# bepu/bepuphysics2

Hardware: NVIDIA B200
Metric: constraint-iterations/sec (solver+integrator) (higher is better)
Workload: dtype f32

## Files before the change

bepuphysics2_b200/csrc/bepu_contacts.cuh:

```cuda
#pragma once
#include "bepu_device_math.cuh"

namespace BEPU_NS {

constexpr int kLanes = 32;

struct GlobalRows { const float* ptr; };
struct GlobalAcc { float* ptr; };
struct StagedRows { uint32_t addr, bar, parity; };
struct StagedAcc { uint32_t addr; float* ptr; };
BEPU_DI float lds_f32(uint32_t addr) {
    float v;
    asm("ld.shared.f32 %0, [%1];" : "=f"(v) : "r"(addr));
    return v;
}
BEPU_DI void rows_ready(GlobalRows) {}
BEPU_DI void rows_ready(StagedRows p) {
    asm volatile(
        "{\n"
        ".reg .pred p;\n"
        "MBAR_WAIT:\n"
        "mbarrier.try_wait.parity.shared::cta.b64 p, [%0], %1;\n"
        "@p bra MBAR_DONE;\n"
        "bra MBAR_WAIT;\n"
// ... 12 lines not shown
BEPU_DI void stacc(StagedAcc a, int r, float v) { __stcs(a.ptr + r * kLanes, v); }

BEPU_DI void penetration_apply(const Inertia& iA, const Inertia& iB, V3 normal, V3 angularA, V3 angularB, float impulse, Velocity& vA, Velocity& vB) {
    V3 dLinA = normal * (impulse * iA.inv_mass);
    V3 dAngA = transform(angularA * impulse, iA.t);
    V3 dLinB = normal * (impulse * iB.inv_mass);
    V3 dAngB = transform(angularB * impulse, iB.t);
    vA.lin = vA.lin + dLinA;
    vA.ang = vA.ang + dAngA;
    vB.lin = vB.lin - dLinB;
    vB.ang = vB.ang + dAngB;
}
BEPU_DI void penetration_warm_start(const Inertia& iA, const Inertia& iB, V3 normal, V3 offsetA, V3 offsetB, float accumulated, Velocity& vA, Velocity& vB) {
    penetration_apply(iA, iB, normal, cross(offsetA, normal), cross(normal, offsetB), accumulated, vA, vB);
}
BEPU_DI void penetration_solve(const Inertia& iA, const Inertia& iB, V3 normal, V3 offsetA, V3 offsetB, float depth, const Springiness& sp, float maxRecovery,
                               float inverseDt, float& accumulated, Velocity& vA, Velocity& vB) {
    V3 angularA = cross(offsetA, normal);
    V3 angularB = cross(normal, offsetB);
    float angularA0 = vector_sandwich(angularA, iA.t);
    float angularB0 = vector_sandwich(angularB, iB.t);
    float linear = iA.inv_mass + iB.inv_mass;
    float effectiveMass = sp.effective_mass_cfm_scale / (linear + angularA0 + angularB0);
    float biasVelocity = fmin_ps(depth * inverseDt, fmin_ps(depth * sp.position_error_to_velocity, maxRecovery));
    float csvaLinear = dot(vA.lin, normal);
    float csvaAngular = dot(vA.ang, angularA);
    float negatedCSVBLinear = dot(vB.lin, normal);
    float csvbAngular = dot(vB.ang, angularB);
    float negatedCSI = accumulated * sp.softness_impulse_scale + (csvaLinear - negatedCSVBLinear + csvaAngular + csvbAngular - biasVelocity) * effectiveMass;
    float previous = accumulated;
    accumulated = fmax_ps(0.0f, accumulated - negatedCSI);
    penetration_apply(iA, iB, normal, angularA, angularB, accumulated - previous, vA, vB);
}
BEPU_DI float updated_depth(float dt, V3 contactOffsetA, V3 offsetB, V3 normal, const Velocity& vA, const Velocity& vB, float depth) {
    V3 contactVelocityA = cross(vA.ang, contactOffsetA) + vA.lin;
    V3 contactOffsetB = contactOffsetA - offsetB;
    V3 contactVelocityB = cross(vB.ang, contactOffsetB) + vB.lin;
    float estimatedDepthChangeVelocity = dot(normal, contactVelocityA - contactVelocityB);
    return depth - estimatedDepthChangeVelocity * dt;
}

BEPU_DI void penetration1_apply(const Inertia& iA, V3 normal, V3 angularA, float impulse, Velocity& vA) {
    V3 dLinA = normal * (impulse * iA.inv_mass);
    V3 dAngA = transform(angularA * impulse, iA.t);
    vA.lin = vA.lin + dLinA;
    vA.ang = vA.ang + dAngA;
}
BEPU_DI void penetration1_solve(const Inertia& iA, V3 normal, V3 offsetA, float depth, const Springiness& sp, float maxRecovery, float inverseDt, float& accumulated,
                                Velocity& vA) {
    V3 angularA = cross(offsetA, normal);
    float angularA0 = vector_sandwich(angularA, iA.t);
    float effectiveMass = sp.effective_mass_cfm_scale / (iA.inv_mass + angularA0);
    float biasVelocity = fmin_ps(depth * inverseDt, fmin_ps(depth * sp.position_error_to_velocity, maxRecovery));
    float csvaLinear = dot(vA.lin, normal);
    float csvaAngular = dot(vA.ang, angularA);
    float negatedCSI = accumulated * sp.softness_impulse_scale + (csvaLinear + csvaAngular - biasVelocity) * effectiveMass;
    float previous = accumulated;
    accumulated = fmax_ps(0.0f, accumulated - negatedCSI);
    penetration1_apply(iA, normal, angularA, accumulated - previous, vA);
}
BEPU_DI float updated_depth1(float dt, V3 contactOffset, V3 normal, const Velocity& v, float depth) {
    V3 contactVelocity = cross(v.ang, contactOffset) + v.lin;
    return depth - dot(normal, contactVelocity) * dt;
}

struct TangentJacobians { M23 linearA, angularA, angularB; };
BEPU_DI TangentJacobians tangent_jacobians(V3 tX, V3 tY, V3 offsetA, V3 offsetB) {
    TangentJacobians j;
    j.linearA = {tX, tY};
    j.angularA = {cross(offsetA, tX), cross(offsetA, tY)};
    j.angularB = {cross(tX, offsetB), cross(tY, offsetB)};
    return j;
}
BEPU_DI void tangent_apply(const TangentJacobians& j, const Inertia& iA, const Inertia& iB, V2 impulse, Velocity& vA, Velocity& vB) {
// ... 120 lines not shown
            V3 offset = ldrow3(p, 4 * i);
            penetration_warm_start(iA, iB, normal, offset, offset - offsetB, ldacc(a, 2 + i), vA, vB);
        }
        twist_apply(normal, iA, iB, ldacc(a, N + 2), vA, vB);
    }
    template <class PR, class AR> BEPU_DI static void solve(const Inertia& iA, const Inertia& iB, float dt, float inverseDt, PR p, AR a, Velocity& vA, Velocity& vB) {
        V3 normal = ldrow3(p, L::kNormal), offsetB = ldrow3(p, L::kOffsetB);
        float friction = ldrow(p, L::kFriction), maxRecovery = ldrow(p, L::kMaxRecovery);
        Springiness sp = compute_springiness(ldrow(p, L::kAngularFrequency), ldrow(p, L::kTwiceDampingRatio), dt);
        if constexpr (N > 1) {
            V3 offs[N];
            float depths[N];
#pragma unroll
            for (int i = 0; i < N; ++i) { offs[i] = ldrow3(p, 4 * i); depths[i] = ldrow(p, 4 * i + 3); }
            const V3 centerA = friction_center<N>(offs, depths);
            float penSum = 0.0f, twistSum = 0.0f;
#pragma unroll 1
            for (int i = 0; i < N; ++i) {
                V3 offset = ldrow3(p, 4 * i);
                float pen = ldacc(a, 2 + i);
                penetration_solve(iA, iB, normal, offset, offset - offsetB, ldrow(p, 4 * i + 3), sp, maxRecovery, inverseDt, pen, vA, vB);
                stacc(a, 2 + i, pen);
                const float lever = pen * distance(centerA, offset);
                penSum = i == 0 ? pen : penSum + pen;
                twistSum = i == 0 ? lever : twistSum + lever;
            }
            V3 x, z;
            build_orthonormal_basis(normal, x, z);
            V2 tangent{ldacc(a, 0), ldacc(a, 1)};
            float twist = ldacc(a, N + 2);
            const float premultiplied = (1.0f / N) * friction;
            tangent_solve(x, z, centerA, centerA - offsetB, iA, iB, premultiplied * penSum, tangent, vA, vB);
            twist_solve(normal, iA, iB, premultiplied * twistSum, twist, vA, vB);
            stacc(a, 0, tangent.x);
            stacc(a, 1, tangent.y);
            stacc(a, N + 2, twist);
        } else
        {
        V3 offs[N];
        float depths[N], pen[N];
#pragma unroll
        for (int i = 0; i < N; ++i) { offs[i] = ldrow3(p, 4 * i); depths[i] = ldrow(p, 4 * i + 3); pen[i] = ldacc(a, 2 + i); }
#pragma unroll
// ... 54 lines not shown
        tangent1_apply(M23{x, z}, M23{cross(centerA, x), cross(centerA, z)}, iA, V2{ldacc(a, 0), ldacc(a, 1)}, vA);
#pragma unroll 1
        for (int i = 0; i < N; ++i) penetration1_apply(iA, normal, cross(ldrow3(p, 4 * i), normal), ldacc(a, 2 + i), vA);
        twist1_apply(normal, iA, ldacc(a, N + 2), vA);
    }
    template <class PR, class AR> BEPU_DI static void solve(const Inertia& iA, float dt, float inverseDt, PR p, AR a, Velocity& vA) {
        V3 normal = ldrow3(p, L::kNormal);
        float friction = ldrow(p, L::kFriction), maxRecovery = ldrow(p, L::kMaxRecovery);
        Springiness sp = compute_springiness(ldrow(p, L::kAngularFrequency), ldrow(p, L::kTwiceDampingRatio), dt);
        if constexpr (N > 1) {
            V3 offs[N];
            float depths[N];
#pragma unroll
            for (int i = 0; i < N; ++i) { offs[i] = ldrow3(p, 4 * i); depths[i] = ldrow(p, 4 * i + 3); }
            const V3 centerA = friction_center<N>(offs, depths);
            float penSum = 0.0f, twistSum = 0.0f;
#pragma unroll 1
            for (int i = 0; i < N; ++i) {
                V3 offset = ldrow3(p, 4 * i);
                float pen = ldacc(a, 2 + i);
                penetration1_solve(iA, normal, offset, ldrow(p, 4 * i + 3), sp, maxRecovery, inverseDt, pen, vA);
                stacc(a, 2 + i, pen);
                const float lever = pen * distance(centerA, offset);
                penSum = i == 0 ? pen : penSum + pen;
                twistSum = i == 0 ? lever : twistSum + lever;
            }
            V3 x, z;
            build_orthonormal_basis(normal, x, z);
            V2 tangent{ldacc(a, 0), ldacc(a, 1)};
            float twist = ldacc(a, N + 2);
            const float premultiplied = (1.0f / N) * friction;
            tangent1_solve(x, z, centerA, iA, premultiplied * penSum, tangent, vA);
            twist1_solve(normal, iA, premultiplied * twistSum, twist, vA);
            stacc(a, 0, tangent.x);
            stacc(a, 1, tangent.y);
            stacc(a, N + 2, twist);
        } else
        {
        V3 offs[N];
        float depths[N], pen[N];
#pragma unroll
        for (int i = 0; i < N; ++i) { offs[i] = ldrow3(p, 4 * i); depths[i] = ldrow(p, 4 * i + 3); pen[i] = ldacc(a, 2 + i); }
#pragma unroll
// ... 139 lines not shown
```

bepuphysics2_b200/csrc/bepu_layout_kernels.h:

```cpp
#pragma once
#include "bepu_device_types.h"

namespace bepucuda {

void launch_split_bodies(const void* raw, int body_count, const BodyBuffers& B, cudaStream_t s);
void launch_merge_bodies(void* raw, int body_count, const BodyBuffers& B, cudaStream_t s);
struct TransposeDesc {
    int32_t* src_refs;
    float* src_prestep;
    float* src_impulses;
    const int32_t* map;
    int32_t src_count;
    int32_t bodies, prestep_rows, impulse_rows;
    int32_t src_bundle_base;
    int32_t flags;
    const int32_t* features_old;
    const int32_t* features_new;
};
constexpr int32_t kDescResidentImpulses = 1, kDescRedistribute = 2;
enum { kTransposeRefs = 1, kTransposePrestep = 2, kTransposeImpulses = 4 };
void launch_transpose_in_all(const DeviceTypeBatch* tbs, const TransposeDesc* descs, const WorkItem* work, int work_count, int W, int what, cudaStream_t s);
void launch_transpose_out_all(const DeviceTypeBatch* tbs, const TransposeDesc* descs, const WorkItem* work, int work_count, int W, int what, cudaStream_t s);
void launch_fill_i32(int32_t* p, size_t n, int32_t v, cudaStream_t s);
void launch_redistribute_impulses(const DeviceTypeBatch* tbs, const TransposeDesc* descs, const WorkItem* work, int work_count, cudaStream_t s);
// ... 12 lines not shown
                           int32_t* error_flag, const TransposeDesc* descs, int W, int32_t* source_bundle_flags, cudaStream_t s);
void launch_collect_stage(const DeviceTypeBatch* tbs, const WorkItem* work, int work_count, const int32_t* bodies_per_type, int stage, const BodyBuffers& B, int32_t* staging,
                          cudaStream_t s);
void launch_apply_stage(const int32_t* staging, int planes, const BodyBuffers& B, cudaStream_t s);
void launch_widen_u8(const uint8_t* in, int32_t* out, size_t n, cudaStream_t s);
void launch_narrow_i32(const int32_t* in, uint8_t* out, size_t n, cudaStream_t s);

void launch_shard_exchange(const uint32_t* pushes, int push_count, int what, const BodyBuffers& B, const ShardPeers& peers, const FrameParams* fp, uint32_t exchange_index,
                           int32_t* error_flag, cudaStream_t s);

void launch_fill_peer_masks(const int32_t* refs, uint32_t* peer_masks, size_t count, const uint8_t* body_masks, int rank, cudaStream_t s);
void launch_boundary_flags(const WorkRecord* records, int count, const int32_t* bodies_per_type, long long peer_delta, uint8_t* flags, cudaStream_t s);

void launch_pack_ref_rows(const WorkRecord* records, int count, int32_t* rows, cudaStream_t s);

constexpr int kLaunchPdl = 1, kLaunchPrefetchRows = 2;
struct SolverLaunchers {
    void (*constraint_stage)(int stage, const WorkRecord* records, const int32_t* ref_rows, int work_count, const BodyBuffers& B, const FrameParams* fp, int launch_flags, cudaStream_t s);
    void (*kinematic_stage)(int stage, const int32_t* kinematics, int count, const BodyBuffers& B, const FrameParams* fp, cudaStream_t s);
    void (*final_pose)(const BodyBuffers& B, const FrameParams* fp, cudaStream_t s);
    void (*constraint_stage_sharded)(int stage, const WorkRecord* records, const int32_t* ref_rows, int work_count, const BodyBuffers& B, const FrameParams* fp, int launch_flags, const ShardPeers& peers,
                                     long long peer_delta, const ShardStage& shard, cudaStream_t s);
};
const SolverLaunchers* get_launchers_bepu_fast();
const SolverLaunchers* get_launchers_bepu_strict();

}
```

bepuphysics2_b200/csrc/bepu_solver_kernels.cu:

```cuda
#include <atomic>
#include "bepu_solver_kernels.cuh"
#include "bepu_layout_kernels.h"

namespace BEPU_NS {

void launch_stage_warm_start_first(const WorkRecord* records, const int32_t* ref_rows, int work_count, const BodyBuffers& B, const FrameParams* fp, int launch_flags, cudaStream_t s);
void launch_stage_warm_start(const WorkRecord* records, const int32_t* ref_rows, int work_count, const BodyBuffers& B, const FrameParams* fp, int launch_flags, cudaStream_t s);
void launch_stage_solve(const WorkRecord* records, const int32_t* ref_rows, int work_count, const BodyBuffers& B, const FrameParams* fp, int launch_flags, cudaStream_t s);
void launch_stage_warm_start_first_sharded(const WorkRecord* records, const int32_t* ref_rows, int work_count, const BodyBuffers& B, const FrameParams* fp, int launch_flags, const ShardPeers& peers, long long peer_delta, const ShardStage& shard, cudaStream_t s);
void launch_stage_warm_start_sharded(const WorkRecord* records, const int32_t* ref_rows, int work_count, const BodyBuffers& B, const FrameParams* fp, int launch_flags, const ShardPeers& peers, long long peer_delta, const ShardStage& shard, cudaStream_t s);
void launch_stage_solve_sharded(const WorkRecord* records, const int32_t* ref_rows, int work_count, const BodyBuffers& B, const FrameParams* fp, int launch_flags, const ShardPeers& peers, long long peer_delta, const ShardStage& shard, cudaStream_t s);

#ifndef BEPU_DEEP_MINB
#define BEPU_DEEP_MINB 12
#endif
constexpr int kDeepBatchBundles = 2400;
template <int STAGE, int MINB>
static void launch_stage_variant(const WorkRecord* records, const int32_t* ref_rows, int work_count, const BodyBuffers& B, const FrameParams* fp, int launch_flags, cudaStream_t s) {
    static std::atomic<bool> carveout_set[64] = {};
    int device = 0;
    cudaGetDevice(&device);
    if (!carveout_set[device & 63]) {
        cudaFuncSetAttribute(constraint_stage_kernel<STAGE, MINB>, cudaFuncAttributePreferredSharedMemoryCarveout, cudaSharedmemCarveoutMaxShared);
        carveout_set[device & 63] = true;
    }
    const unsigned blocks = (unsigned)(((size_t)work_count * 32 + kStageBlockThreads - 1) / kStageBlockThreads);
    cudaLaunchConfig_t cfg{};
    cfg.gridDim = dim3(blocks);
    cfg.blockDim = dim3(kStageBlockThreads);
    cfg.dynamicSmemBytes = 0;
    cfg.stream = s;
    cudaLaunchAttribute attr[1];
    attr[0].id = cudaLaunchAttributeProgrammaticStreamSerialization;
    attr[0].val.programmaticStreamSerializationAllowed = 1;
    cfg.attrs = attr;
    cfg.numAttrs = (launch_flags & bepucuda::kLaunchPdl) ? 1 : 0;
    cudaLaunchKernelEx(&cfg, constraint_stage_kernel<STAGE, MINB>, records, ref_rows, work_count, B, fp, (launch_flags & bepucuda::kLaunchPrefetchRows) ? kStagePrefetchRows : 0);
}
template <int STAGE, int MINB>
static void launch_stage_variant_sharded(const WorkRecord* records, const int32_t* ref_rows, int work_count, const BodyBuffers& B, const FrameParams* fp, int launch_flags, const ShardPeers& peers, long long peer_delta,
                                         const ShardStage& shard, cudaStream_t s) {
    static std::atomic<bool> carveout_set[64] = {};
    int device = 0;
    cudaGetDevice(&device);
    if (!carveout_set[device & 63]) {
        cudaFuncSetAttribute(constraint_stage_kernel_sharded<STAGE, MINB>, cudaFuncAttributePreferredSharedMemoryCarveout, cudaSharedmemCarveoutMaxShared);
        carveout_set[device & 63] = true;
    }
    const unsigned blocks = (unsigned)(((size_t)work_count * 32 + kStageBlockThreads - 1) / kStageBlockThreads);
    cudaLaunchConfig_t cfg{};
    cfg.gridDim = dim3(blocks);
    cfg.blockDim = dim3(kStageBlockThreads);
// ... 88 lines not shown
```

bepuphysics2_b200/csrc/bepu_solver_kernels.cuh:

```cuda
#pragma once
#include "bepu_contacts.cuh"
#include "bepu_joints_more.cuh"
#include "bepu_integration.cuh"
#include "bepu_device_types.h"

namespace BEPU_NS {

using namespace bepucuda;

struct F8 { float a, b, c, d, e, f, g, h; };
#define BEPU_BODY_LD "ld.global.L1::no_allocate.L2::evict_last.v8.f32"
#define BEPU_BODY_ST "st.global.L1::no_allocate.L2::evict_last.v8.f32"
BEPU_DI F8 ld256(const float4* p) {
    F8 r;
    asm volatile(BEPU_BODY_LD " {%0,%1,%2,%3,%4,%5,%6,%7}, [%8];"
                 : "=f"(r.a), "=f"(r.b), "=f"(r.c), "=f"(r.d), "=f"(r.e), "=f"(r.f), "=f"(r.g), "=f"(r.h)
                 : "l"(p)
                 : "memory");
    return r;
}
BEPU_DI void st256(float4* p, float a, float b, float c, float d, float e, float f, float g, float h) {
    asm volatile(BEPU_BODY_ST " [%0], {%1,%2,%3,%4,%5,%6,%7,%8};" ::"l"(p), "f"(a), "f"(b), "f"(c), "f"(d), "f"(e), "f"(f), "f"(g), "f"(h) : "memory");
}
BEPU_DI void load_velocity(const float4* vel, uint32_t i, Velocity& v) {
// ... 3 lines not shown
}
BEPU_DI void store_velocity(float4* vel, uint32_t i, const Velocity& v) { st256(vel + 2 * (size_t)i, v.lin.x, v.lin.y, v.lin.z, 0.0f, v.ang.x, v.ang.y, v.ang.z, 0.0f); }
BEPU_DI void load_inertia(const float4* in, uint32_t i, Inertia& r) {
    const F8 x = ld256(in + 2 * (size_t)i);
    r.t = {x.a, x.b, x.c, x.d, x.e, x.f};
    r.inv_mass = x.g;
}
BEPU_DI void store_inertia(float4* in, uint32_t i, const Inertia& r) { st256(in + 2 * (size_t)i, r.t.xx, r.t.yx, r.t.yy, r.t.zx, r.t.zy, r.t.zz, r.inv_mass, 0.0f); }
BEPU_DI void load_pose(const float4* pose, uint32_t i, V3& pos, Q4& q) {
    const F8 x = ld256(pose + 2 * (size_t)i);
    q = {x.a, x.b, x.c, x.d};
    pos = {x.e, x.f, x.g};
}
BEPU_DI void store_pose(float4* pose, uint32_t i, V3 pos, Q4 q) { st256(pose + 2 * (size_t)i, q.x, q.y, q.z, q.w, pos.x, pos.y, pos.z, 0.0f); }

template <int STAGE, bool NeedsPose>
BEPU_DI void warm_start_body(uint32_t enc, const BodyBuffers& B, const FrameParams& fp, BodyState& b, Velocity& v) {
    const uint32_t idx = enc & kRefIndexMask;
    if (enc & kRefIntegrateBit) {
        Inertia local;
        load_inertia(B.inertia_local, idx, local);
        load_pose(B.pose, idx, b.pos, b.q);
        b.inertia.inv_mass = local.inv_mass;
        if (STAGE == kStageWarmStart) {
            b.pos = b.pos + v.lin * fp.dt;
            Q4 previousOrientation = b.q;
            b.q = integrate_orientation(b.q, v.ang, fp.dt * 0.5f);
            b.inertia.t = rotate_inverse_inertia(local.t, b.q);
            if (fp.angular_mode == 1) integrate_angular_conserve_momentum(previousOrientation, local.t, b.inertia.t, v.ang);
            else if (fp.angular_mode == 2) integrate_angular_gyroscopic(b.q, local.t, v.ang, fp.dt);
            store_pose(B.pose, idx, b.pos, b.q);
        } else {
            b.inertia.t = rotate_inverse_inertia(local.t, b.q);
            if (fp.angular_mode == 1) {
                Q4 previousOrientation = integrate_orientation(b.q, v.ang, fp.dt * -0.5f);
                integrate_angular_conserve_momentum(previousOrientation, local.t, b.inertia.t, v.ang);
            } else if (fp.angular_mode == 2) {
// ... 5 lines not shown
    } else {
        load_inertia(B.inertia_world, idx, b.inertia);
        if (NeedsPose) load_pose(B.pose, idx, b.pos, b.q);
        if (STAGE == kStageWarmStartFirst && fp.angular_mode != 0 && (enc & kRefBundleIntegratesBit) && !(enc & kRefKinematicBit)) {
            Inertia local;
            load_inertia(B.inertia_local, idx, local);
            V3 pos;
            Q4 q;
            load_pose(B.pose, idx, pos, q);
            if (fp.angular_mode == 1) integrate_angular_conserve_momentum(integrate_orientation(q, v.ang, fp.dt * -0.5f), local.t, b.inertia.t, v.ang);
            else integrate_angular_gyroscopic(q, local.t, v.ang, fp.dt);
        }
    }
}
template <int STAGE, bool NeedsPose>
BEPU_DI void gather_for_warm_start(uint32_t enc, const BodyBuffers& B, const FrameParams& fp, BodyState& b, Velocity& v) {
    load_velocity(B.velocity, enc & kRefIndexMask, v);
    warm_start_body<STAGE, NeedsPose>(enc, B, fp, b, v);
}

template <class T, class PR, class AR> BEPU_DI void call_warm_start(const BodyState* b, PR p, AR a, Velocity* v) {
    if constexpr (T::kNeedsPose) T::warm_start(b, p, a, v);
    else if constexpr (T::kBodies == 2) T::warm_start(b[0].inertia, b[1].inertia, p, a, v[0], v[1]);
    else T::warm_start(b[0].inertia, p, a, v[0]);
}
template <class T, class PR, class AR> BEPU_DI void call_solve(const BodyState* b, float dt, float inverseDt, PR p, AR a, Velocity* v) {
    if constexpr (T::kNeedsPose) T::solve(b, dt, inverseDt, p, a, v);
    else if constexpr (T::kBodies == 2) T::solve(b[0].inertia, b[1].inertia, dt, inverseDt, p, a, v[0], v[1]);
    else T::solve(b[0].inertia, dt, inverseDt, p, a, v[0]);
}
template <class T> BEPU_DI void call_incremental(float dt, const Velocity* v, float* p) {
    if constexpr (T::kIncremental) {
        if constexpr (T::kBodies == 2) T::incremental_update(dt, v[0], v[1], p);
// ... 4 lines not shown
BEPU_DI uint32_t ldg_nc_u32(const void* p) {
    uint32_t v;
    asm volatile("ld.global.nc.u32 %0, [%1];" : "=r"(v) : "l"(p));
    return v;
}
BEPU_DI void push_record(float4* const* arrays, uint32_t mask, uint32_t idx, float a, float b, float c, float d, float e, float f, float g, float h) {
    while (mask) {
        const int q = __ffs((int)mask) - 1;
        mask &= mask - 1u;
        float4* dst = arrays[q] + 2 * (size_t)idx;
        dst[0] = make_float4(a, b, c, d);
        dst[1] = make_float4(e, f, g, h);
    }
}
template <class T, int STAGE, bool kSharded, class PR, class AR>
BEPU_DI void run_lane(const int32_t* refs, PR p, AR a, float* p_rw, uint32_t enc0, uint32_t enc1, const BodyBuffers& B, const FrameParams& fp, const ShardPeers* peers = nullptr,
                      long long peer_delta = 0) {
    constexpr int NB = T::kBodies;
    uint32_t enc[NB];
    enc[0] = enc0;
    if constexpr (NB > 1) enc[1] = enc1;
#pragma unroll
    for (int s = 2; s < NB; ++s) enc[s] = (uint32_t)__ldg(refs + s * kLanes);
    uint32_t push_to[kSharded ? NB : 1];
    if constexpr (kSharded) {
#pragma unroll
        for (int s = 0; s < NB; ++s) push_to[s] = peer_delta != 0 ? ldg_nc_u32(refs + peer_delta + s * kLanes) : 0u;
    }
    if ((int32_t)enc[0] == kRefEmpty) return;
    BodyState b[NB];
    Velocity v[NB];
    if constexpr (STAGE == kStageIncremental) {
#pragma unroll
        for (int s = 0; s < NB; ++s) load_velocity(B.velocity, enc[s] & kRefIndexMask, v[s]);
        call_incremental<T>(fp.dt, v, p_rw);
    } else if constexpr (STAGE == kStageSolve) {
#pragma unroll
        for (int s = 0; s < NB; ++s) {
            const uint32_t idx = enc[s] & kRefIndexMask;
            load_velocity(B.velocity, idx, v[s]);
            load_inertia(B.inertia_world, idx, b[s].inertia);
            if (T::kNeedsPose) load_pose(B.pose, idx, b[s].pos, b[s].q);
        }
        rows_ready(p);
        call_solve<T>(b, fp.dt, fp.inverse_dt, p, a, v);
#pragma unroll
        for (int s = 0; s < NB; ++s)
            if (!(enc[s] & kRefKinematicBit)) {
                store_velocity(B.velocity, enc[s] & kRefIndexMask, v[s]);
                if constexpr (kSharded) {
                    const uint32_t mask = push_to[s];
                    if (mask) push_record(peers->velocity, mask, enc[s] & kRefIndexMask, v[s].lin.x, v[s].lin.y, v[s].lin.z, 0.0f, v[s].ang.x, v[s].ang.y, v[s].ang.z, 0.0f);
                }
            }
    } else {
#pragma unroll
        for (int s = 0; s < NB; ++s) gather_for_warm_start<STAGE, T::kNeedsPose>(enc[s], B, fp, b[s], v[s]);
        rows_ready(p);
        call_warm_start<T>(b, p, a, v);
#pragma unroll
        for (int s = 0; s < NB; ++s)
            if (!(enc[s] & kRefKinematicBit)) {
                const uint32_t idx = enc[s] & kRefIndexMask;
                store_velocity(B.velocity, idx, v[s]);
                if constexpr (kSharded) {
                    const uint32_t mask = push_to[s];
                    if (mask) {
                        push_record(peers->velocity, mask, idx, v[s].lin.x, v[s].lin.y, v[s].lin.z, 0.0f, v[s].ang.x, v[s].ang.y, v[s].ang.z, 0.0f);
                        if (enc[s] & kRefIntegrateBit) {
                            const Inertia& in = b[s].inertia;
                            push_record(peers->inertia_world, mask, idx, in.t.xx, in.t.yx, in.t.yy, in.t.zx, in.t.zy, in.t.zz, in.inv_mass, 0.0f);
                            if (STAGE == kStageWarmStart) push_record(peers->pose, mask, idx, b[s].q.x, b[s].q.y, b[s].q.z, b[s].q.w, b[s].pos.x, b[s].pos.y, b[s].pos.z, 0.0f);
                        }
                    }
                }
            }
    }
}
template <class T, int STAGE, class PR, class AR>
BEPU_DI void run_lane(const int32_t* refs, PR p, AR a, float* p_rw, uint32_t enc0, uint32_t enc1, const BodyBuffers& B, const FrameParams& fp) {
    run_lane<T, STAGE, false>(refs, p, a, p_rw, enc0, enc1, B, fp);
}

BEPU_DI int4 ldg_nc_v4(const void* p) {
    int4 v;
    asm volatile("ld.global.nc.v4.s32 {%0,%1,%2,%3}, [%4];" : "=r"(v.x), "=r"(v.y), "=r"(v.z), "=r"(v.w) : "l"(p));
    return v;
}
BEPU_DI WorkRecord load_record(const WorkRecord* r) {
    const int4 lo = ldg_nc_v4(r), hi = ldg_nc_v4(reinterpret_cast<const int4*>(r) + 1);
    WorkRecord w;
    w.refs = reinterpret_cast<int32_t*>((unsigned long long)(unsigned int)lo.x | ((unsigned long long)(unsigned int)lo.y << 32));
    w.prestep = reinterpret_cast<float*>((unsigned long long)(unsigned int)lo.z | ((unsigned long long)(unsigned int)lo.w << 32));
    w.impulses = reinterpret_cast<float*>((unsigned long long)(unsigned int)hi.x | ((unsigned long long)(unsigned int)hi.y << 32));
    w.type_id = hi.z;
    w.live_lanes = hi.w;
    return w;
}

#define BEPU_CONTACT_TYPES(X)                                                                                                     \
    X(0, ConvexOneBody<1>) X(1, ConvexOneBody<2>) X(2, ConvexOneBody<3>) X(3, ConvexOneBody<4>)                                   \
    X(4, ConvexTwoBody<1>) X(5, ConvexTwoBody<2>) X(6, ConvexTwoBody<3>) X(7, ConvexTwoBody<4>)                                   \
    X(8, NonconvexOneBody<2>) X(9, NonconvexOneBody<3>) X(10, NonconvexOneBody<4>)                                                \
    X(15, NonconvexTwoBody<2>) X(16, NonconvexTwoBody<3>) X(17, NonconvexTwoBody<4>)

template <int STAGE, bool kSharded, class PR, class AR>
BEPU_DI void run_bundle_rows(const WorkRecord& rec, int lane, PR p, AR a, uint32_t enc0, uint32_t enc1, const BodyBuffers& B, const FrameParams& fp, const ShardPeers* peers = nullptr,
                             long long peer_delta = 0) {
    const int32_t* refs = rec.refs + lane;
    float* p_rw = rec.prestep + lane;
    switch (rec.type_id) {
#define BEPU_CASE(ID, T) \
    case ID: run_lane<T, STAGE, kSharded>(refs, p, a, p_rw, enc0, enc1, B, fp, peers, peer_delta); break;
        BEPU_CONTACT_TYPES(BEPU_CASE)
        BEPU_JOINT_TYPES(BEPU_CASE)
        BEPU_JOINT_TYPES_MORE(BEPU_CASE)
#undef BEPU_CASE
        default: break;
    }
}
template <int STAGE, class PR, class AR>
BEPU_DI void run_bundle_rows(const WorkRecord& rec, int lane, PR p, AR a, uint32_t enc0, uint32_t enc1, const BodyBuffers& B, const FrameParams& fp) {
    run_bundle_rows<STAGE, false>(rec, lane, p, a, enc0, enc1, B, fp);
}
template <int STAGE>
BEPU_DI void run_bundle(const WorkRecord& rec, int lane, uint32_t enc0, uint32_t enc1, const BodyBuffers& B, const FrameParams& fp) {
    run_bundle_rows<STAGE>(rec, lane, GlobalRows{rec.prestep + lane}, GlobalAcc{rec.impulses + lane}, enc0, enc1, B, fp);
}
template <int STAGE> BEPU_DI void run_bundle(const WorkRecord& rec, int lane, const BodyBuffers& B, const FrameParams& fp) {
    const uint32_t enc0 = ldg_nc_u32(rec.refs + lane), enc1 = ldg_nc_u32(rec.refs + kLanes + lane);
    run_bundle<STAGE>(rec, lane, enc0, enc1, B, fp);
}

struct StageRowCounts { uint8_t prestep[64], impulses[64]; };
__host__ __device__ constexpr StageRowCounts make_stage_row_counts() {
    StageRowCounts c{};
#define BEPU_ROWS(ID, T) c.prestep[ID] = (uint8_t)T::kPrestepRows; c.impulses[ID] = (uint8_t)T::kImpulseRows;
    BEPU_CONTACT_TYPES(BEPU_ROWS)
    BEPU_JOINT_TYPES(BEPU_ROWS)
    BEPU_JOINT_TYPES_MORE(BEPU_ROWS)
#undef BEPU_ROWS
    return c;
}
__constant__ StageRowCounts kStageRowCounts = make_stage_row_counts();
constexpr int kStageSlabRows = 48;
constexpr int kStageSlabBytes = kStageSlabRows * kLanes * 4;

BEPU_DI uint32_t smem_u32(const void* p) { return (uint32_t)__cvta_generic_to_shared(p); }
BEPU_DI void mbar_init(uint32_t bar, uint32_t count) {
    asm volatile("mbarrier.init.shared::cta.b64 [%0], %1;" ::"r"(bar), "r"(count) : "memory");
    asm volatile("fence.mbarrier_init.release.cluster;" ::: "memory");
    asm volatile("fence.proxy.async.shared::cta;" ::: "memory");
// ... 3 lines not shown
    uint64_t policy;
    asm volatile("createpolicy.fractional.L2::evict_first.b64 %0, 1.0;" : "=l"(policy));
    return policy;
}
BEPU_DI void bulk_copy_g2s(uint32_t dst, const void* src, uint32_t bytes, uint32_t bar, uint64_t policy) {
    asm volatile("cp.async.bulk.shared::cluster.global.mbarrier::complete_tx::bytes.L2::cache_hint [%0], [%1], %2, [%3], %4;" ::"r"(dst), "l"(src), "r"(bytes), "r"(bar),
                 "l"(policy)
                 : "memory");
}

#ifndef BEPU_STAGE_BLOCK_THREADS
#define BEPU_STAGE_BLOCK_THREADS 64
#endif
constexpr int kStageBlockThreads = BEPU_STAGE_BLOCK_THREADS;

constexpr int kStagePrefetchRows = 1;
BEPU_DI void shard_announce(const ShardPeers& peers, int lane) {
    if (lane < peers.rank_count && lane != peers.rank)
        asm volatile("red.release.sys.global.add.u64 [%0], 1;" ::"l"(peers.flags[lane] + kShardCounterSlot + peers.rank) : "memory");
}
BEPU_DI void shard_wait(const ShardPeers& peers, int lane, uint32_t solve_index, uint32_t exchange_point, int32_t* error_flag) {
    if (lane < peers.rank_count && lane != peers.rank) {
        const unsigned long long* mine = peers.flags[peers.rank];
        const unsigned long long* targets = mine + kShardTargetSlot + (size_t)lane * kShardMaxExchanges;
        const unsigned long long want = (unsigned long long)solve_index * targets[kShardMaxExchanges - 1] + targets[exchange_point];
        unsigned long long seen;
        unsigned int spins = 0;
        do {
            asm volatile("ld.acquire.sys.global.u64 %0, [%1];" : "=l"(seen) : "l"(mine + kShardCounterSlot + lane) : "memory");
        } while (seen < want && ++spins < 100000000u);
        if (seen < want) atomicExch(error_flag, 5);
    }
    __syncwarp();
}
template <int STAGE, bool kSharded>
BEPU_DI void constraint_stage_body(const WorkRecord* __restrict__ records, const int32_t* __restrict__ ref_rows, int work_count, const BodyBuffers& B, const FrameParams* __restrict__ fpp, int flags, const ShardPeers* peers,
                                   long long peer_delta, const ShardStage* shard = nullptr) {
    constexpr bool kStaged = STAGE != kStageIncremental;
    constexpr int kWarps = kStageBlockThreads / 32;
    __shared__ __align__(128) float slab[kStaged ? kWarps * kStageSlabRows * kLanes : 1];
    __shared__ __align__(8) unsigned long long bars[kWarps];
    const int warp_in_block = threadIdx.x >> 5;
    const int global_warp = (blockIdx.x * kStageBlockThreads + threadIdx.x) >> 5;
    const int lane = threadIdx.x & 31;
    WorkRecord rec{};
    uint32_t enc0 = (uint32_t)kRefEmpty, enc1 = 0;
    const int warp = global_warp;
    const bool active = warp < work_count;
    const uint32_t slab_addr = kStaged ? smem_u32(slab) + warp_in_block * kStageSlabBytes : 0;
    const uint32_t bar = smem_u32(&bars[warp_in_block]);
    const bool early_rows = kStaged && (flags & kStagePrefetchRows);
    uint32_t prestep_bytes = 0, impulse_bytes = 0;
    if (active) {
        rec = load_record(records + warp);
        if constexpr (kStaged) {
            prestep_bytes = kStageRowCounts.prestep[rec.type_id] * (kLanes * 4);
            impulse_bytes = kStageRowCounts.impulses[rec.type_id] * (kLanes * 4);
            if (lane == 0) {
                mbar_init(bar, 1);
                if (early_rows) {
                    const uint64_t policy = l2_evict_first_policy();
                    mbar_expect_tx(bar, prestep_bytes + impulse_bytes);
                    bulk_copy_g2s(slab_addr, rec.prestep, prestep_bytes, bar, policy);
                    bulk_copy_g2s(slab_addr + prestep_bytes, rec.impulses, impulse_bytes, bar, policy);
                }
            }
        }
        enc0 = ldg_nc_u32(ref_rows + (size_t)warp * (2 * kLanes) + lane);
        enc1 = ldg_nc_u32(ref_rows + (size_t)warp * (2 * kLanes) + kLanes + lane);
    }
    const FrameParams fp = *fpp;
    asm volatile("griddepcontrol.wait;" ::: "memory");
    asm volatile("griddepcontrol.launch_dependents;");
    bool boundary = false;
    if constexpr (kSharded) {
        boundary = active && (rec.live_lanes & kRecordBoundaryBit) != 0;
        if (boundary && shard->exchange_index > 0 && !(fp.tune[0] & 1)) shard_wait(*peers, lane, fp.shard_solve_index, shard->exchange_index - 1u, shard->error_flag);
    }
    if (!active) return;
    if constexpr (kStaged) {
        if (!early_rows && lane == 0) {
            const uint64_t policy = l2_evict_first_policy();
            mbar_expect_tx(bar, prestep_bytes + impulse_bytes);
            bulk_copy_g2s(slab_addr, rec.prestep, prestep_bytes, bar, policy);
            bulk_copy_g2s(slab_addr + prestep_bytes, rec.impulses, impulse_bytes, bar, policy);
        }
        __syncwarp();
        run_bundle_rows<STAGE, kSharded>(rec, lane, StagedRows{slab_addr + lane * 4, bar, 0u}, StagedAcc{slab_addr + prestep_bytes + lane * 4, rec.impulses + lane}, enc0, enc1, B, fp,
                                         peers, boundary && !(fp.tune[0] & 4) ? peer_delta : 0);
        if constexpr (kSharded) {
            if (boundary && !(fp.tune[0] & 2)) {
                __syncwarp();
                shard_announce(*peers, lane);
            }
        }
    } else {
        run_bundle<STAGE>(rec, lane, enc0, enc1, B, fp);
    }
}

template <int STAGE, int MINB>
__global__ void __launch_bounds__(kStageBlockThreads, MINB) constraint_stage_kernel(const WorkRecord* __restrict__ records, const int32_t* __restrict__ ref_rows, int work_count, BodyBuffers B, const FrameParams* __restrict__ fpp, int flags) {
    constraint_stage_body<STAGE, false>(records, ref_rows, work_count, B, fpp, flags, nullptr, 0);
}
// ... 76 lines not shown
```

bepuphysics2_b200/csrc/bepucuda_api.cu:

```cuda
#include <algorithm>
#include <cmath>
#include <cstdio>
#include <cstdlib>
#include <cstring>
#include <map>
#include <string>
#include <vector>

#include "../../include/bepucuda.h"
#include "bepu_layout_kernels.h"
#include "bepu_coloring.h"
#include "bepu_bounds.h"
#include "bepu_shape_bounds.h"

using namespace bepucuda;

namespace bepucuda {

static TypeInfo make_contact(int bodies, int prestep, int impulses, int contacts, const char* name) {
    TypeInfo t{};
    t.bodies = bodies; t.prestep_rows = prestep; t.impulse_rows = impulses; t.incremental = 1; t.name = name;
    const int body_rw = 13 + 6;
    t.solve_bytes = 4 * (prestep + 2 * impulses + bodies + bodies * body_rw);
    t.warm_start_bytes = 4 * (prestep + impulses + bodies + bodies * body_rw);
// ... 311 lines not shown
                ++n;
            }
            if (fused_pushes) { ++exchange_index; continue; }
            const auto& range = ctx->push_range[op.pad - 2];
            launch_shard_exchange(ctx->pushes_dev.as<uint32_t>() + range.first, range.second, op.stage == kStageSolve ? 1 : (op.stage == kStageWarmStart ? 3 : 2), ctx->B, ctx->peers, fp,
                                  exchange_index++, ctx->error_dev.as<int32_t>(), s);
            ++n;
            if (op.work_count > 0) previous = &op;
            continue;
        }
        switch (op.stage) {
            case kStageWarmStartFirst: case kStageWarmStart: case kStageSolve: case kStageIncremental:
                if (op.work_count > 0) {
                    bool prefetch = op.stage != kStageIncremental && previous != nullptr && previous->stage != kStageIncremental;
                    if (prefetch && previous->stage <= kStageSolve && previous->work_begin == op.work_begin) prefetch = false;
                    if (ctx->exchange) {
                        ctx->launchers->constraint_stage(op.stage, records + op.work_begin, ref_rows + (size_t)op.work_begin * 64, op.work_count, ctx->B, fp, 0, s);
                        ++n;
                        if (op.stage != kStageIncremental) {
                            const int planes = op.stage == kStageSolve ? 1 : (op.stage == kStageWarmStart ? 3 : 2);
                            const size_t words = (size_t)ctx->body_count * 8 * planes;
                            cudaMemsetAsync(ctx->exchange_staging.ptr, 0, words * 4, s);
                            launch_collect_stage(ctx->tb_table.as<DeviceTypeBatch>(), ctx->work_table.as<WorkItem>() + op.work_begin, op.work_count, ctx->bodies_per_type.as<int32_t>(), op.stage,
                                                 ctx->B, ctx->exchange_staging.as<int32_t>(), s);
                            if (ctx->exchange(ctx->exchange_user, ctx->exchange_staging.ptr, (int64_t)words, 0, (void*)s) != 0) ctx->exchange_failed = true;
                            launch_apply_stage(ctx->exchange_staging.as<int32_t>(), planes, ctx->B, s);
                            n += 2;
                        }
                        previous = &op;
                        break;
                    }
                    ctx->launchers->constraint_stage(op.stage, records + op.work_begin, ref_rows + (size_t)op.work_begin * 64, op.work_count, ctx->B, fp, (pdl ? kLaunchPdl : 0) | (prefetch ? kLaunchPrefetchRows : 0), s);
                    previous = &op;
                    ++n;
                }
                break;
            case kStageKinematicFirst: case kStageKinematic:
                if (op.work_count > 0) { ctx->launchers->kinematic_stage(op.stage, kin, op.work_count, ctx->B, fp, s); previous = &op; ++n; }
                break;
            case kStageFinalPose:
                if (ctx->B.count > 0) { ctx->launchers->final_pose(ctx->B, fp, s); previous = &op; ++n; }
                break;
        }
    }
    if (launches) *launches = n;
    ctx->exchanges_per_solve = exchange_index;
}
// ... 1394 lines not shown
```

Measured before the change: 3.825 billion.

## Prefetch body inertia/pose before PDL wait and software-pipeline contact penetration rows

```diff
diff --git a/bepuphysics2_b200/csrc/bepu_contacts.cuh b/bepuphysics2_b200/csrc/bepu_contacts.cuh
--- a/bepuphysics2_b200/csrc/bepu_contacts.cuh
+++ b/bepuphysics2_b200/csrc/bepu_contacts.cuh
@@ -50,23 +50,32 @@
 BEPU_DI void penetration_warm_start(const Inertia& iA, const Inertia& iB, V3 normal, V3 offsetA, V3 offsetB, float accumulated, Velocity& vA, Velocity& vB) {
     penetration_apply(iA, iB, normal, cross(offsetA, normal), cross(normal, offsetB), accumulated, vA, vB);
 }
+struct PenetrationRow { V3 angularA, angularB; float effectiveMass, biasVelocity; };
+BEPU_DI PenetrationRow penetration_row(const Inertia& iA, const Inertia& iB, V3 normal, V3 offsetA, V3 offsetB, float depth, const Springiness& sp, float maxRecovery,
+                                       float inverseDt) {
+    PenetrationRow r;
+    r.angularA = cross(offsetA, normal);
+    r.angularB = cross(normal, offsetB);
+    float angularA0 = vector_sandwich(r.angularA, iA.t);
+    float angularB0 = vector_sandwich(r.angularB, iB.t);
+    float linear = iA.inv_mass + iB.inv_mass;
+    r.effectiveMass = sp.effective_mass_cfm_scale / (linear + angularA0 + angularB0);
+    r.biasVelocity = fmin_ps(depth * inverseDt, fmin_ps(depth * sp.position_error_to_velocity, maxRecovery));
+    return r;
+}
+BEPU_DI void penetration_solve(const Inertia& iA, const Inertia& iB, V3 normal, const PenetrationRow& r, const Springiness& sp, float& accumulated, Velocity& vA, Velocity& vB) {
+    float csvaLinear = dot(vA.lin, normal);
+    float csvaAngular = dot(vA.ang, r.angularA);
+    float negatedCSVBLinear = dot(vB.lin, normal);
+    float csvbAngular = dot(vB.ang, r.angularB);
+    float negatedCSI = accumulated * sp.softness_impulse_scale + (csvaLinear - negatedCSVBLinear + csvaAngular + csvbAngular - r.biasVelocity) * r.effectiveMass;
+    float previous = accumulated;
+    accumulated = fmax_ps(0.0f, accumulated - negatedCSI);
+    penetration_apply(iA, iB, normal, r.angularA, r.angularB, accumulated - previous, vA, vB);
+}
 BEPU_DI void penetration_solve(const Inertia& iA, const Inertia& iB, V3 normal, V3 offsetA, V3 offsetB, float depth, const Springiness& sp, float maxRecovery,
                                float inverseDt, float& accumulated, Velocity& vA, Velocity& vB) {
-    V3 angularA = cross(offsetA, normal);
-    V3 angularB = cross(normal, offsetB);
-    float angularA0 = vector_sandwich(angularA, iA.t);
-    float angularB0 = vector_sandwich(angularB, iB.t);
-    float linear = iA.inv_mass + iB.inv_mass;
-    float effectiveMass = sp.effective_mass_cfm_scale / (linear + angularA0 + angularB0);
-    float biasVelocity = fmin_ps(depth * inverseDt, fmin_ps(depth * sp.position_error_to_velocity, maxRecovery));
-    float csvaLinear = dot(vA.lin, normal);
-    float csvaAngular = dot(vA.ang, angularA);
-    float negatedCSVBLinear = dot(vB.lin, normal);
-    float csvbAngular = dot(vB.ang, angularB);
-    float negatedCSI = accumulated * sp.softness_impulse_scale + (csvaLinear - negatedCSVBLinear + csvaAngular + csvbAngular - biasVelocity) * effectiveMass;
-    float previous = accumulated;
-    accumulated = fmax_ps(0.0f, accumulated - negatedCSI);
-    penetration_apply(iA, iB, normal, angularA, angularB, accumulated - previous, vA, vB);
+    penetration_solve(iA, iB, normal, penetration_row(iA, iB, normal, offsetA, offsetB, depth, sp, maxRecovery, inverseDt), sp, accumulated, vA, vB);
 }
 BEPU_DI float updated_depth(float dt, V3 contactOffsetA, V3 offsetB, V3 normal, const Velocity& vA, const Velocity& vB, float depth) {
     V3 contactVelocityA = cross(vA.ang, contactOffsetA) + vA.lin;
@@ -82,18 +91,26 @@
     vA.lin = vA.lin + dLinA;
     vA.ang = vA.ang + dAngA;
 }
+struct PenetrationRow1 { V3 angularA; float effectiveMass, biasVelocity; };
+BEPU_DI PenetrationRow1 penetration1_row(const Inertia& iA, V3 normal, V3 offsetA, float depth, const Springiness& sp, float maxRecovery, float inverseDt) {
+    PenetrationRow1 r;
+    r.angularA = cross(offsetA, normal);
+    float angularA0 = vector_sandwich(r.angularA, iA.t);
+    r.effectiveMass = sp.effective_mass_cfm_scale / (iA.inv_mass + angularA0);
+    r.biasVelocity = fmin_ps(depth * inverseDt, fmin_ps(depth * sp.position_error_to_velocity, maxRecovery));
+    return r;
+}
+BEPU_DI void penetration1_solve(const Inertia& iA, V3 normal, const PenetrationRow1& r, const Springiness& sp, float& accumulated, Velocity& vA) {
+    float csvaLinear = dot(vA.lin, normal);
+    float csvaAngular = dot(vA.ang, r.angularA);
+    float negatedCSI = accumulated * sp.softness_impulse_scale + (csvaLinear + csvaAngular - r.biasVelocity) * r.effectiveMass;
+    float previous = accumulated;
+    accumulated = fmax_ps(0.0f, accumulated - negatedCSI);
+    penetration1_apply(iA, normal, r.angularA, accumulated - previous, vA);
+}
 BEPU_DI void penetration1_solve(const Inertia& iA, V3 normal, V3 offsetA, float depth, const Springiness& sp, float maxRecovery, float inverseDt, float& accumulated,
                                 Velocity& vA) {
-    V3 angularA = cross(offsetA, normal);
-    float angularA0 = vector_sandwich(angularA, iA.t);
-    float effectiveMass = sp.effective_mass_cfm_scale / (iA.inv_mass + angularA0);
-    float biasVelocity = fmin_ps(depth * inverseDt, fmin_ps(depth * sp.position_error_to_velocity, maxRecovery));
-    float csvaLinear = dot(vA.lin, normal);
-    float csvaAngular = dot(vA.ang, angularA);
-    float negatedCSI = accumulated * sp.softness_impulse_scale + (csvaLinear + csvaAngular - biasVelocity) * effectiveMass;
-    float previous = accumulated;
-    accumulated = fmax_ps(0.0f, accumulated - negatedCSI);
-    penetration1_apply(iA, normal, angularA, accumulated - previous, vA);
+    penetration1_solve(iA, normal, penetration1_row(iA, normal, offsetA, depth, sp, maxRecovery, inverseDt), sp, accumulated, vA);
 }
 BEPU_DI float updated_depth1(float dt, V3 contactOffset, V3 normal, const Velocity& v, float depth) {
     V3 contactVelocity = cross(v.ang, contactOffset) + v.lin;
@@ -244,19 +261,26 @@
 #pragma unroll
             for (int i = 0; i < N; ++i) { offs[i] = ldrow3(p, 4 * i); depths[i] = ldrow(p, 4 * i + 3); }
             const V3 centerA = friction_center<N>(offs, depths);
+            V3 x, z;
+            build_orthonormal_basis(normal, x, z);
+            PenetrationRow row = penetration_row(iA, iB, normal, offs[0], offs[0] - offsetB, depths[0], sp, maxRecovery, inverseDt);
+            float leverArm = distance(centerA, offs[0]);
             float penSum = 0.0f, twistSum = 0.0f;
 #pragma unroll 1
             for (int i = 0; i < N; ++i) {
-                V3 offset = ldrow3(p, 4 * i);
+                const int k = i + 1 < N ? i + 1 : i;
+                const V3 nextOffset = ldrow3(p, 4 * k);
+                const PenetrationRow next = penetration_row(iA, iB, normal, nextOffset, nextOffset - offsetB, ldrow(p, 4 * k + 3), sp, maxRecovery, inverseDt);
+                const float nextLeverArm = distance(centerA, nextOffset);
                 float pen = ldacc(a, 2 + i);
-                penetration_solve(iA, iB, normal, offset, offset - offsetB, ldrow(p, 4 * i + 3), sp, maxRecovery, inverseDt, pen, vA, vB);
+                penetration_solve(iA, iB, normal, row, sp, pen, vA, vB);
                 stacc(a, 2 + i, pen);
-                const float lever = pen * distance(centerA, offset);
+                const float lever = pen * leverArm;
                 penSum = i == 0 ? pen : penSum + pen;
                 twistSum = i == 0 ? lever : twistSum + lever;
+                row = next;
+                leverArm = nextLeverArm;
             }
-            V3 x, z;
-            build_orthonormal_basis(normal, x, z);
             V2 tangent{ldacc(a, 0), ldacc(a, 1)};
             float twist = ldacc(a, N + 2);
             const float premultiplied = (1.0f / N) * friction;
@@ -341,19 +365,26 @@
 #pragma unroll
             for (int i = 0; i < N; ++i) { offs[i] = ldrow3(p, 4 * i); depths[i] = ldrow(p, 4 * i + 3); }
             const V3 centerA = friction_center<N>(offs, depths);
+            V3 x, z;
+            build_orthonormal_basis(normal, x, z);
+            PenetrationRow1 row = penetration1_row(iA, normal, offs[0], depths[0], sp, maxRecovery, inverseDt);
+            float leverArm = distance(centerA, offs[0]);
             float penSum = 0.0f, twistSum = 0.0f;
 #pragma unroll 1
             for (int i = 0; i < N; ++i) {
-                V3 offset = ldrow3(p, 4 * i);
+                const int k = i + 1 < N ? i + 1 : i;
+                const V3 nextOffset = ldrow3(p, 4 * k);
+                const PenetrationRow1 next = penetration1_row(iA, normal, nextOffset, ldrow(p, 4 * k + 3), sp, maxRecovery, inverseDt);
+                const float nextLeverArm = distance(centerA, nextOffset);
                 float pen = ldacc(a, 2 + i);
-                penetration1_solve(iA, normal, offset, ldrow(p, 4 * i + 3), sp, maxRecovery, inverseDt, pen, vA);
+                penetration1_solve(iA, normal, row, sp, pen, vA);
                 stacc(a, 2 + i, pen);
-                const float lever = pen * distance(centerA, offset);
+                const float lever = pen * leverArm;
                 penSum = i == 0 ? pen : penSum + pen;
                 twistSum = i == 0 ? lever : twistSum + lever;
+                row = next;
+                leverArm = nextLeverArm;
             }
-            V3 x, z;
-            build_orthonormal_basis(normal, x, z);
             V2 tangent{ldacc(a, 0), ldacc(a, 1)};
             float twist = ldacc(a, N + 2);
             const float premultiplied = (1.0f / N) * friction;
diff --git a/bepuphysics2_b200/csrc/bepu_layout_kernels.h b/bepuphysics2_b200/csrc/bepu_layout_kernels.h
--- a/bepuphysics2_b200/csrc/bepu_layout_kernels.h
+++ b/bepuphysics2_b200/csrc/bepu_layout_kernels.h
@@ -50,7 +50,7 @@
 
 void launch_pack_ref_rows(const WorkRecord* records, int count, int32_t* rows, cudaStream_t s);
 
-constexpr int kLaunchPdl = 1, kLaunchPrefetchRows = 2;
+constexpr int kLaunchPdl = 1, kLaunchPrefetchRows = 2, kLaunchPrefetchBodies = 4;
 struct SolverLaunchers {
     void (*constraint_stage)(int stage, const WorkRecord* records, const int32_t* ref_rows, int work_count, const BodyBuffers& B, const FrameParams* fp, int launch_flags, cudaStream_t s);
     void (*kinematic_stage)(int stage, const int32_t* kinematics, int count, const BodyBuffers& B, const FrameParams* fp, cudaStream_t s);
diff --git a/bepuphysics2_b200/csrc/bepu_solver_kernels.cu b/bepuphysics2_b200/csrc/bepu_solver_kernels.cu
--- a/bepuphysics2_b200/csrc/bepu_solver_kernels.cu
+++ b/bepuphysics2_b200/csrc/bepu_solver_kernels.cu
@@ -35,7 +35,8 @@
     attr[0].val.programmaticStreamSerializationAllowed = 1;
     cfg.attrs = attr;
     cfg.numAttrs = (launch_flags & bepucuda::kLaunchPdl) ? 1 : 0;
-    cudaLaunchKernelEx(&cfg, constraint_stage_kernel<STAGE, MINB>, records, ref_rows, work_count, B, fp, (launch_flags & bepucuda::kLaunchPrefetchRows) ? kStagePrefetchRows : 0);
+    const int flags = ((launch_flags & bepucuda::kLaunchPrefetchRows) ? kStagePrefetchRows : 0) | ((launch_flags & bepucuda::kLaunchPrefetchBodies) ? kStagePrefetchBodies : 0);
+    cudaLaunchKernelEx(&cfg, constraint_stage_kernel<STAGE, MINB>, records, ref_rows, work_count, B, fp, flags);
 }
 template <int STAGE, int MINB>
 static void launch_stage_variant_sharded(const WorkRecord* records, const int32_t* ref_rows, int work_count, const BodyBuffers& B, const FrameParams* fp, int launch_flags, const ShardPeers& peers, long long peer_delta,
diff --git a/bepuphysics2_b200/csrc/bepu_solver_kernels.cuh b/bepuphysics2_b200/csrc/bepu_solver_kernels.cuh
--- a/bepuphysics2_b200/csrc/bepu_solver_kernels.cuh
+++ b/bepuphysics2_b200/csrc/bepu_solver_kernels.cuh
@@ -41,13 +41,30 @@
 }
 BEPU_DI void store_pose(float4* pose, uint32_t i, V3 pos, Q4 q) { st256(pose + 2 * (size_t)i, q.x, q.y, q.z, q.w, pos.x, pos.y, pos.z, 0.0f); }
 
+struct BodyRecords {
+    Inertia inertia;
+    V3 pos;
+    Q4 q;
+};
+template <int STAGE>
+BEPU_DI void load_body_records(uint32_t enc, bool needs_pose, const BodyBuffers& B, BodyRecords& r) {
+    const uint32_t idx = enc & kRefIndexMask;
+    if constexpr (STAGE == kStageSolve) {
+        load_inertia(B.inertia_world, idx, r.inertia);
+        if (needs_pose) load_pose(B.pose, idx, r.pos, r.q);
+    } else if (enc & kRefIntegrateBit) {
+        load_inertia(B.inertia_local, idx, r.inertia);
+        load_pose(B.pose, idx, r.pos, r.q);
+    }
+}
+
 template <int STAGE, bool NeedsPose>
-BEPU_DI void warm_start_body(uint32_t enc, const BodyBuffers& B, const FrameParams& fp, BodyState& b, Velocity& v) {
+BEPU_DI void warm_start_body(uint32_t enc, const BodyRecords& r, const BodyBuffers& B, const FrameParams& fp, BodyState& b, Velocity& v) {
     const uint32_t idx = enc & kRefIndexMask;
     if (enc & kRefIntegrateBit) {
-        Inertia local;
-        load_inertia(B.inertia_local, idx, local);
-        load_pose(B.pose, idx, b.pos, b.q);
+        const Inertia local = r.inertia;
+        b.pos = r.pos;
+        b.q = r.q;
         b.inertia.inv_mass = local.inv_mass;
         if (STAGE == kStageWarmStart) {
             b.pos = b.pos + v.lin * fp.dt;
@@ -83,9 +100,9 @@
     }
 }
 template <int STAGE, bool NeedsPose>
-BEPU_DI void gather_for_warm_start(uint32_t enc, const BodyBuffers& B, const FrameParams& fp, BodyState& b, Velocity& v) {
+BEPU_DI void gather_for_warm_start(uint32_t enc, const BodyRecords& r, const BodyBuffers& B, const FrameParams& fp, BodyState& b, Velocity& v) {
     load_velocity(B.velocity, enc & kRefIndexMask, v);
-    warm_start_body<STAGE, NeedsPose>(enc, B, fp, b, v);
+    warm_start_body<STAGE, NeedsPose>(enc, r, B, fp, b, v);
 }
 
 template <class T, class PR, class AR> BEPU_DI void call_warm_start(const BodyState* b, PR p, AR a, Velocity* v) {
@@ -120,8 +137,8 @@
     }
 }
 template <class T, int STAGE, bool kSharded, class PR, class AR>
-BEPU_DI void run_lane(const int32_t* refs, PR p, AR a, float* p_rw, uint32_t enc0, uint32_t enc1, const BodyBuffers& B, const FrameParams& fp, const ShardPeers* peers = nullptr,
-                      long long peer_delta = 0) {
+BEPU_DI void run_lane(const int32_t* refs, PR p, AR a, float* p_rw, uint32_t enc0, uint32_t enc1, const BodyRecords (&pre)[2], const BodyBuffers& B, const FrameParams& fp,
+                      const ShardPeers* peers = nullptr, long long peer_delta = 0) {
     constexpr int NB = T::kBodies;
     uint32_t enc[NB];
     enc[0] = enc0;
@@ -143,10 +160,15 @@
     } else if constexpr (STAGE == kStageSolve) {
 #pragma unroll
         for (int s = 0; s < NB; ++s) {
-            const uint32_t idx = enc[s] & kRefIndexMask;
-            load_velocity(B.velocity, idx, v[s]);
-            load_inertia(B.inertia_world, idx, b[s].inertia);
-            if (T::kNeedsPose) load_pose(B.pose, idx, b[s].pos, b[s].q);
+            load_velocity(B.velocity, enc[s] & kRefIndexMask, v[s]);
+            BodyRecords r;
+            if (s < 2) r = pre[s];
+            else load_body_records<STAGE>(enc[s], T::kNeedsPose, B, r);
+            b[s].inertia = r.inertia;
+            if (T::kNeedsPose) {
+                b[s].pos = r.pos;
+                b[s].q = r.q;
+            }
         }
         rows_ready(p);
         call_solve<T>(b, fp.dt, fp.inverse_dt, p, a, v);
@@ -161,7 +183,12 @@
             }
     } else {
 #pragma unroll
-        for (int s = 0; s < NB; ++s) gather_for_warm_start<STAGE, T::kNeedsPose>(enc[s], B, fp, b[s], v[s]);
+        for (int s = 0; s < NB; ++s) {
+            BodyRecords r;
+            if (s < 2) r = pre[s];
+            else load_body_records<STAGE>(enc[s], T::kNeedsPose, B, r);
+            gather_for_warm_start<STAGE, T::kNeedsPose>(enc[s], r, B, fp, b[s], v[s]);
+        }
         rows_ready(p);
         call_warm_start<T>(b, p, a, v);
 #pragma unroll
@@ -184,8 +211,8 @@
     }
 }
 template <class T, int STAGE, class PR, class AR>
-BEPU_DI void run_lane(const int32_t* refs, PR p, AR a, float* p_rw, uint32_t enc0, uint32_t enc1, const BodyBuffers& B, const FrameParams& fp) {
-    run_lane<T, STAGE, false>(refs, p, a, p_rw, enc0, enc1, B, fp);
+BEPU_DI void run_lane(const int32_t* refs, PR p, AR a, float* p_rw, uint32_t enc0, uint32_t enc1, const BodyRecords (&pre)[2], const BodyBuffers& B, const FrameParams& fp) {
+    run_lane<T, STAGE, false>(refs, p, a, p_rw, enc0, enc1, pre, B, fp);
 }
 
 BEPU_DI int4 ldg_nc_v4(const void* p) {
@@ -211,13 +238,13 @@
     X(15, NonconvexTwoBody<2>) X(16, NonconvexTwoBody<3>) X(17, NonconvexTwoBody<4>)
 
 template <int STAGE, bool kSharded, class PR, class AR>
-BEPU_DI void run_bundle_rows(const WorkRecord& rec, int lane, PR p, AR a, uint32_t enc0, uint32_t enc1, const BodyBuffers& B, const FrameParams& fp, const ShardPeers* peers = nullptr,
-                             long long peer_delta = 0) {
+BEPU_DI void run_bundle_rows(const WorkRecord& rec, int lane, PR p, AR a, uint32_t enc0, uint32_t enc1, const BodyRecords (&pre)[2], const BodyBuffers& B, const FrameParams& fp,
+                             const ShardPeers* peers = nullptr, long long peer_delta = 0) {
     const int32_t* refs = rec.refs + lane;
     float* p_rw = rec.prestep + lane;
     switch (rec.type_id) {
 #define BEPU_CASE(ID, T) \
-    case ID: run_lane<T, STAGE, kSharded>(refs, p, a, p_rw, enc0, enc1, B, fp, peers, peer_delta); break;
+    case ID: run_lane<T, STAGE, kSharded>(refs, p, a, p_rw, enc0, enc1, pre, B, fp, peers, peer_delta); break;
         BEPU_CONTACT_TYPES(BEPU_CASE)
         BEPU_JOINT_TYPES(BEPU_CASE)
         BEPU_JOINT_TYPES_MORE(BEPU_CASE)
@@ -226,22 +253,28 @@
     }
 }
 template <int STAGE, class PR, class AR>
-BEPU_DI void run_bundle_rows(const WorkRecord& rec, int lane, PR p, AR a, uint32_t enc0, uint32_t enc1, const BodyBuffers& B, const FrameParams& fp) {
-    run_bundle_rows<STAGE, false>(rec, lane, p, a, enc0, enc1, B, fp);
+BEPU_DI void run_bundle_rows(const WorkRecord& rec, int lane, PR p, AR a, uint32_t enc0, uint32_t enc1, const BodyRecords (&pre)[2], const BodyBuffers& B, const FrameParams& fp) {
+    run_bundle_rows<STAGE, false>(rec, lane, p, a, enc0, enc1, pre, B, fp);
 }
 template <int STAGE>
 BEPU_DI void run_bundle(const WorkRecord& rec, int lane, uint32_t enc0, uint32_t enc1, const BodyBuffers& B, const FrameParams& fp) {
-    run_bundle_rows<STAGE>(rec, lane, GlobalRows{rec.prestep + lane}, GlobalAcc{rec.impulses + lane}, enc0, enc1, B, fp);
+    static_assert(STAGE == kStageIncremental, "the staged stages take their body records from constraint_stage_body");
+    const BodyRecords unused[2] = {};
+    run_bundle_rows<STAGE>(rec, lane, GlobalRows{rec.prestep + lane}, GlobalAcc{rec.impulses + lane}, enc0, enc1, unused, B, fp);
 }
 template <int STAGE> BEPU_DI void run_bundle(const WorkRecord& rec, int lane, const BodyBuffers& B, const FrameParams& fp) {
     const uint32_t enc0 = ldg_nc_u32(rec.refs + lane), enc1 = ldg_nc_u32(rec.refs + kLanes + lane);
     run_bundle<STAGE>(rec, lane, enc0, enc1, B, fp);
 }
 
-struct StageRowCounts { uint8_t prestep[64], impulses[64]; };
+constexpr uint8_t kTypeSecondBody = 1, kTypeNeedsPose = 2;
+struct StageRowCounts { uint8_t prestep[64], impulses[64], body_flags[64]; };
 __host__ __device__ constexpr StageRowCounts make_stage_row_counts() {
     StageRowCounts c{};
-#define BEPU_ROWS(ID, T) c.prestep[ID] = (uint8_t)T::kPrestepRows; c.impulses[ID] = (uint8_t)T::kImpulseRows;
+#define BEPU_ROWS(ID, T)                                  \
+    c.prestep[ID] = (uint8_t)T::kPrestepRows;             \
+    c.impulses[ID] = (uint8_t)T::kImpulseRows;            \
+    c.body_flags[ID] = (uint8_t)((T::kBodies > 1 ? kTypeSecondBody : 0) | (T::kNeedsPose ? kTypeNeedsPose : 0));
     BEPU_CONTACT_TYPES(BEPU_ROWS)
     BEPU_JOINT_TYPES(BEPU_ROWS)
     BEPU_JOINT_TYPES_MORE(BEPU_ROWS)
@@ -275,7 +308,7 @@
 #endif
 constexpr int kStageBlockThreads = BEPU_STAGE_BLOCK_THREADS;
 
-constexpr int kStagePrefetchRows = 1;
+constexpr int kStagePrefetchRows = 1, kStagePrefetchBodies = 2;
 BEPU_DI void shard_announce(const ShardPeers& peers, int lane) {
     if (lane < peers.rank_count && lane != peers.rank)
         asm volatile("red.release.sys.global.add.u64 [%0], 1;" ::"l"(peers.flags[lane] + kShardCounterSlot + peers.rank) : "memory");
@@ -293,6 +326,13 @@
         if (seen < want) atomicExch(error_flag, 5);
     }
     __syncwarp();
+}
+template <int STAGE>
+BEPU_DI void load_slot_records(uint32_t enc0, uint32_t enc1, uint32_t type_flags, const BodyBuffers& B, BodyRecords (&r)[2]) {
+    if ((int32_t)enc0 == kRefEmpty) return;
+    const bool needs_pose = (type_flags & kTypeNeedsPose) != 0;
+    load_body_records<STAGE>(enc0, needs_pose, B, r[0]);
+    if (type_flags & kTypeSecondBody) load_body_records<STAGE>(enc1, needs_pose, B, r[1]);
 }
 template <int STAGE, bool kSharded>
 BEPU_DI void constraint_stage_body(const WorkRecord* __restrict__ records, const int32_t* __restrict__ ref_rows, int work_count, const BodyBuffers& B, const FrameParams* __restrict__ fpp, int flags, const ShardPeers* peers,
@@ -311,12 +351,15 @@
     const uint32_t slab_addr = kStaged ? smem_u32(slab) + warp_in_block * kStageSlabBytes : 0;
     const uint32_t bar = smem_u32(&bars[warp_in_block]);
     const bool early_rows = kStaged && (flags & kStagePrefetchRows);
-    uint32_t prestep_bytes = 0, impulse_bytes = 0;
+    const bool early_bodies = kStaged && !kSharded && (flags & kStagePrefetchBodies);
+    uint32_t prestep_bytes = 0, impulse_bytes = 0, type_flags = 0;
+    BodyRecords pre[2];
     if (active) {
         rec = load_record(records + warp);
         if constexpr (kStaged) {
             prestep_bytes = kStageRowCounts.prestep[rec.type_id] * (kLanes * 4);
             impulse_bytes = kStageRowCounts.impulses[rec.type_id] * (kLanes * 4);
+            type_flags = kStageRowCounts.body_flags[rec.type_id];
             if (lane == 0) {
                 mbar_init(bar, 1);
                 if (early_rows) {
@@ -329,6 +372,7 @@
         }
         enc0 = ldg_nc_u32(ref_rows + (size_t)warp * (2 * kLanes) + lane);
         enc1 = ldg_nc_u32(ref_rows + (size_t)warp * (2 * kLanes) + kLanes + lane);
+        if (early_bodies) load_slot_records<STAGE>(enc0, enc1, type_flags, B, pre);
     }
     const FrameParams fp = *fpp;
     asm volatile("griddepcontrol.wait;" ::: "memory");
@@ -346,9 +390,10 @@
             bulk_copy_g2s(slab_addr, rec.prestep, prestep_bytes, bar, policy);
             bulk_copy_g2s(slab_addr + prestep_bytes, rec.impulses, impulse_bytes, bar, policy);
         }
+        if (!early_bodies) load_slot_records<STAGE>(enc0, enc1, type_flags, B, pre);
         __syncwarp();
-        run_bundle_rows<STAGE, kSharded>(rec, lane, StagedRows{slab_addr + lane * 4, bar, 0u}, StagedAcc{slab_addr + prestep_bytes + lane * 4, rec.impulses + lane}, enc0, enc1, B, fp,
-                                         peers, boundary && !(fp.tune[0] & 4) ? peer_delta : 0);
+        run_bundle_rows<STAGE, kSharded>(rec, lane, StagedRows{slab_addr + lane * 4, bar, 0u}, StagedAcc{slab_addr + prestep_bytes + lane * 4, rec.impulses + lane}, enc0, enc1, pre, B,
+                                         fp, peers, boundary && !(fp.tune[0] & 4) ? peer_delta : 0);
         if constexpr (kSharded) {
             if (boundary && !(fp.tune[0] & 2)) {
                 __syncwarp();
diff --git a/bepuphysics2_b200/csrc/bepucuda_api.cu b/bepuphysics2_b200/csrc/bepucuda_api.cu
--- a/bepuphysics2_b200/csrc/bepucuda_api.cu
+++ b/bepuphysics2_b200/csrc/bepucuda_api.cu
@@ -349,6 +349,8 @@
                 if (op.work_count > 0) {
                     bool prefetch = op.stage != kStageIncremental && previous != nullptr && previous->stage != kStageIncremental;
                     if (prefetch && previous->stage <= kStageSolve && previous->work_begin == op.work_begin) prefetch = false;
+                    const bool after_constraints = !ctx->peer_mode && !ctx->exchange && previous != nullptr && previous->stage <= kStageIncremental;
+                    const bool prefetch_bodies = op.stage == kStageSolve ? after_constraints && previous->stage >= kStageSolve : op.stage != kStageIncremental && after_constraints;
                     if (ctx->exchange) {
                         ctx->launchers->constraint_stage(op.stage, records + op.work_begin, ref_rows + (size_t)op.work_begin * 64, op.work_count, ctx->B, fp, 0, s);
                         ++n;
@@ -365,7 +367,7 @@
                         previous = &op;
                         break;
                     }
-                    ctx->launchers->constraint_stage(op.stage, records + op.work_begin, ref_rows + (size_t)op.work_begin * 64, op.work_count, ctx->B, fp, (pdl ? kLaunchPdl : 0) | (prefetch ? kLaunchPrefetchRows : 0), s);
+                    ctx->launchers->constraint_stage(op.stage, records + op.work_begin, ref_rows + (size_t)op.work_begin * 64, op.work_count, ctx->B, fp, (pdl ? kLaunchPdl : 0) | (prefetch ? kLaunchPrefetchRows : 0) | (prefetch_bodies ? kLaunchPrefetchBodies : 0), s);
                     previous = &op;
                     ++n;
                 }
```

Result: no change. 3.816 billion (median of 6 runs) (-0.2%).
